# Yuliang-Eliott/Alpha-Multi-factor-models

Measured on AMD Instinct MI355X. Metric: asset-days/sec, factor build+XS regression+KKT (10k assets x 20y), 1/2/4/8 GPU, higher is better.
Workload: dtype f64

## Files before the change

alpha-multi-factor-models_amd/afm/_lib.py:

```python
from __future__ import annotations

import contextlib
import ctypes
import operator
import os
import threading

HERE = os.path.dirname(os.path.abspath(__file__))
LIB_PATH = os.environ.get("AFM_LIB") or os.path.join(HERE, "libafm.so")

P = ctypes.c_void_p
I64 = ctypes.c_int64
I32 = ctypes.c_int
DBL = ctypes.c_double

SIGNATURES = {
    "afm_ctx_create": ("status", "int ptr"),
    "afm_ctx_set_stream": ("status", "ctx ptr"),
    "afm_ctx_set_option": ("status", "ctx str i64"),
    "afm_ctx_get_option": ("status", "ctx str host:i64*"),
    "afm_stream_create_cu_mask": ("status", "int ptr int ptr"),
    "afm_stream_destroy": ("status", "ptr"),
    "afm_ctx_destroy": ("status", "ctx"),
    "afm_last_error": ("str", ""),
# ... 15 lines not shown
    "afm_drop_last_obs_bits_range": ("status", "ctx i64 i64 i64* i64* i64* i64 i64"),
    "afm_factors_part_words": ("i64", "ctx i64 i64 i64 i64"),
    "afm_factors_range_part_f64": ("status", "ctx i64 i64 i64 i64 i64 f64* f64* i64* f64* f64* "
                                             "i64*"),
    "afm_factor_masks_f64": ("status", "ctx i64 i64 i64 i64 i64 i64* i64* i64* i64*"),
    "afm_predict_f64": ("status", "ctx f64* i64 i64 i64 i64 i32* int f64* i64 i64* int f64*"),
    "afm_fama_macbeth_f64": ("status", "ctx f64* i32* i64 int f64* f64*"),
    "afm_ols_residual_f64": ("status", "ctx f64* i64 int int f64* f64* f64*"),
    "afm_vec_add_f64": ("status", "ctx i64 f64* f64*"),
    "afm_ols_intercept_f64": ("status", "ctx int f64* f64*"),
    "afm_lasso_cd_f64": ("status", "ctx f64* int f64 f64 int f64 int f64* f64*"),
    "afm_talib_factors_f64": ("status", "ctx i64 i64 i64 f64* f64* i64* f64*"),
    "afm_ffill_f64": ("status", "ctx i64 i64 i64 f64* i64*"),
    "afm_date_mean_fill_f64": ("status", "ctx i64 i64 i64 i64 f64* i64* f64*"),
    "afm_group_demean_f64": ("status", "ctx i64 i64* i64 f64* f64* f64*"),
    "afm_rebalance_f64": ("status", "ctx i64 i64 i64 i32* i64 f64* i64* f64* i64* i64 i64 i64 f64* "
                                    "f64* int f64 f64 i32* i32* f64* f64* i32* i64* i32*"),
    "afm_pnl_scan_f64": ("status", "ctx i64 i32* i32* f64* i32* i64* f64 f64 f64* f64* f64* f64*"),
    "afm_bootstrap_pnl_f64": ("status", "ctx i64 i32* i64 f64* i32* i32* f64* i64 i64 i32* f64 f64 "
                                        "f64* f64* f64* f64*"),
    "afm_min_variance_weights_f64": ("status", "ctx f64* i64 i64 int f64 f64 f64* f64* i32*"),
    "afm_fwd_returns_f64": ("status", "ctx i64 i64 f64* i64* f64*"),
    "afm_xs_prepare_f64": ("status", "ctx i64 i64 i64 f64* f64* f64* f64* i32* i32*"),
    "afm_xs_prepare_range_f64": ("status", "ctx i64 i64 i64 i64 i64 f64* f64* f64* f64* i32* i32*"),
    "afm_xs_rank_f64": ("status", "ctx i64 i64 f64* i32* i64* i32* i32* i32*"),
    "afm_xs_layers_f64": ("status", "ctx i64 i64 f64* i32* i64* i32* i32* i32*"),
    "afm_xs_stats_f64": ("status", "ctx i64 i64 i32* i64 f64* i32* i32* i32* int f64* f64* i32* "
                                   "f64*"),
    "afm_xs_series_f64": ("status", "ctx i64 f64* f64* f64* i32* int int f64* f64* f64* f64* f64*"),
    "afm_zscore_stats_f64": ("status", "ctx f64* i64 i64 i64 i32* int i64* i64 i64 f64* f64*"),
    "afm_zscore_stats_slab_f64": ("status", "ctx f64* i64 i64 i64 i32* int i64* i64 i64 f64* int "
                                            "int f64* f64*"),
    "afm_zscore_apply_f64": ("status", "ctx f64* i64 i64 i64 i32* int i64* i64 i64 f64* f64* f64* "
                                       "i64 i32* i64*"),
    "afm_zgram_part_bytes": ("int", "int"),
    "afm_zstats_finalize_f64": ("status", "ctx f64* f64* int i64 f64* i32*"),
    "afm_row_bits": ("status", "ctx i64 i64 i64* i64* i32* i64 i64 i64*"),
    "afm_zgram_f64": ("status", "ctx f64* i64 i64 i32* i32* int int f64* int i64* i64 i64 int i64 "
                                "i64 i64 f64* int"),
    "afm_zpool_f64": ("status", "ctx f64* i64 i64 i32* i32* int int f64* int i64* i64 i64 i64 int "
                                "i64 int f64* int"),
    "afm_gram_tree_f64": ("status", "ctx int f64* i64 int int f64*"),
    "afm_zpredict_f64": ("status", "ctx f64* i64 i64 i64 i64 i32* int f64* f64* i64* f64*"),
    "afm_lasso_fit_f64": ("status", "ctx f64* f64* int f64 int f64 int f64* f64*"),
    "afm_lasso_batch_f64": ("status", "ctx f64* i64 f64* i64 int f64* int i64 int int f64 int f64* "
                                      "f64*"),
    "afm_gram_score_f64": ("status", "ctx f64* i64 f64* i64 int f64* int i64 f64*"),
}
SIGNATURES_MV = {
    "afm_rebalance_mv_f64": ("status", "ctx i64 i64 i64 i32* i64 f64* i64* f64* i64* i64 i64 i64 "
                                       "f64* f64* int f64 f64 f64* f64 i32* i32* f64* f64* i32* "
                                       "i64* i32*"),
    "afm_mean_variance_weights_f64": ("status", "ctx f64* i64 i64 int f64* f64 f64 f64 f64* f64* "
                                                "i32*"),
}
SIGNATURES_SCREEN = {
    "afm_screen_ic_f64": ("status", "ctx f64* i64 i64 i64 i32* int f64* i32* i32* i64 f64* i32* "
                                    "i32* f64*"),
    "afm_screen_summary_f64": ("status", "ctx f64* i64 int i32* int int f64* f64* f64*"),
}
TABLES = (SIGNATURES, SIGNATURES_MV, SIGNATURES_SCREEN)
SIGNATURES_RANK = {
    "afm_rank_scratch_words": ("i64", "i64"),
    "afm_rank_returns_f64": ("status", "ctx i64 i64 i32* i64 f64* i32* i32* i64* i64*"),
    "afm_screen_rank_ic_f64": ("status", "ctx f64* i64 i64 i64 i32* int f64* i32* i32* i64 f64* "
                                         "i32* i32* i32* i64* i64* f64*"),
}
ALL_TABLES = TABLES + (SIGNATURES_RANK,)
SIGNATURES_SEAMS = {
    "afm_gram_tree3_f64": ("status", "ctx int f64* int int int int int f64*"),
    "afm_gram_final_f64": ("status", "ctx int f64* int f64* int f64* f64*"),
    "afm_ols_solve_parts_f64": ("status", "ctx f64* int f64* int i64 f64 f64* f64* i32*"),
    "afm_factors_rows_f64": ("status", "ctx i64 i64 i64 f64* f64* f64* f64* i64* f64* i64* i64* "
                                       "i64* i64*"),
    "afm_zstats_rows_f64": ("status", "ctx f64* f64* int i64 f64* i32* i64 i64* i64 i64 i64*"),
}
LOADED_TABLES = ALL_TABLES + (SIGNATURES_SEAMS,)
SIGNATURES_LAYERS = {
    "afm_screen_layers_f64": ("status", "ctx f64* i64 i64 i64 i32* int f64* i32* i32* i64 f64* i32* "
                                        "i32* f64* i32* f64* f64*"),
    "afm_screen_layer_series_f64": ("status", "ctx i64 int f64* f64* f64* f64* f64*"),
}
BOUND_TABLES = LOADED_TABLES + (SIGNATURES_LAYERS,)
_RESTYPE = {"status": I32, "int": I32, "i64": I64, "str": ctypes.c_char_p}
_ARGTYPE = {"int": I32, "i64": I64, "f64": DBL, "str": ctypes.c_char_p}


class AfmError(RuntimeError):
    pass


_lib = None
_lock = threading.Lock()


def lib():
    global _lib
    if _lib is None:
        with _lock:
            if _lib is None:
                if not os.path.exists(LIB_PATH):
                    raise ImportError(f"{LIB_PATH} is not built: run `make -C "
                                      f"{os.path.dirname(HERE)}` (hipcc, gfx950)")
                L = ctypes.CDLL(LIB_PATH)
                for table in BOUND_TABLES:
                    for name, (res, params) in table.items():
                        f = getattr(L, name)
                        f.restype = _RESTYPE[res]
                        f.argtypes = [_ARGTYPE.get(t, P) for t in params.split()]
                _lib = L
    return _lib


def check(rc: int, what: str = ""):
    if rc != 0:
        msg = lib().afm_last_error().decode(errors="replace")
        raise AfmError(f"{what or 'afm'} failed ({rc}): {msg}")


def _as_given(a):
    return a


def _device_buffer(dtype, device: int, where: str):
    import torch

    def conv(t):
        if t is None:
            return None
        if not isinstance(t, torch.Tensor):
            raise AfmError(f"{where}: expected a {dtype} tensor or None, got {type(t).__name__}")
        if t.get_device() != device or t.dtype is not dtype or not t.is_contiguous():
            raise AfmError(f"{where}: expected a contiguous {dtype} tensor on cuda:{device}, got "
                           f"{t.dtype} on {t.device}, contiguous={t.is_contiguous()}")
        return t.data_ptr()
    return conv


def _plans(device: int) -> dict:
    import torch
    scalar = {"int": operator.index, "i64": operator.index, "f64": float}
    buffer = {"f64*": torch.float64, "i32*": torch.int32, "i64*": torch.int64}
    negative = (0).__gt__
    failed = {"status": bool, "int": negative, "i64": negative, "str": lambda s: s is None}
    plans = {}
    for name, (res, params) in (item for table in BOUND_TABLES for item in table.items()):
        toks = params.split()
        takes_ctx = toks[:1] == ["ctx"]
        convs = tuple(_device_buffer(buffer[t], device, f"{name} argument {i}") if t in buffer
                      else scalar.get(t, _as_given)
                      for i, t in enumerate(toks[takes_ctx:], 1))
        plans[name] = (takes_ctx, convs, failed[res])
    return plans


class Context:

    _by_device: dict = {}

    def __init__(self, device: int):
        self.device = device
        h = P()
        check(lib().afm_ctx_create(device, ctypes.byref(h)), "afm_ctx_create")
        self.handle = h
        self._plans = _plans(device)

    def call(self, name: str, *args):
        takes_ctx, convs, failed = self._plans[name]
        if len(args) != len(convs):
            raise TypeError(f"{name} takes {len(convs)} arguments ({len(args)} given)")
        cargs = [cv(a) for cv, a in zip(convs, args)]
        fn = getattr(lib(), name)
        rc = fn(self.handle, *cargs) if takes_ctx else fn(*cargs)
        if failed(rc):
            raise AfmError(f"{name} failed ({rc}): "
                           f"{lib().afm_last_error().decode(errors='replace')}")
        return rc

    @classmethod
    def get(cls, device: int | None = None) -> "Context":
        import torch
        if not torch.cuda.is_available():
            raise AfmError("no GPU visible: the afm engine runs on MI355X only (no CPU fallback)")
        if device is None:
            device = torch.cuda.current_device()
        ctx = cls._by_device.get(device)
        if ctx is None:
            ctx = cls._by_device[device] = Context(device)
        return ctx

    def set_option(self, name: str, value: int):
        self.call("afm_ctx_set_option", name.encode(), int(value))

    def get_option(self, name: str) -> int:
        v = I64()
        self.call("afm_ctx_get_option", name.encode(), ctypes.byref(v))
        return int(v.value)

    def bind_stream(self):
        import torch
        s = torch.cuda.current_stream(self.device).cuda_stream
        check(lib().afm_ctx_set_stream(self.handle, P(s)), "afm_ctx_set_stream")
        return self.handle

    @contextlib.contextmanager
    def on(self, stream):
        import torch
        try:
            with torch.cuda.stream(stream):
                yield self.bind_stream()
        finally:
            self.bind_stream()


def ptr(t) -> P:
    if not t.is_contiguous():
        raise AfmError("tensor must be contiguous")
    return P(t.data_ptr())


def run(name: str, *args, device: int | None = None):
    if device is None:
        device = next((a.device.index for a in args if hasattr(a, "data_ptr")), None)
    ctx = Context.get(device)
    ctx.bind_stream()
    return ctx.call(name, *args)


def factor_names() -> list:
# ... 54 lines not shown
```

alpha-multi-factor-models_amd/csrc/zgram.hip:

```cpp
#include "afm_internal.h"
#include "afm_seams.h"
#include "zgram_layout.h"

#include <cstdlib>

#pragma clang fp contract(off)

namespace afm {
namespace {

typedef double d4 __attribute__((ext_vector_type(4)));
typedef unsigned long long u64;
typedef __attribute__((address_space(3))) double lds_double;

constexpr int kZRS = 66;
constexpr int kZMaxSlots = 3;
constexpr int kZLds = 160 * 1024 - 256;
constexpr int kZProd = 8;
constexpr int kZThreads = 13 * 64;
#ifndef AFM_ZG2_NCW
#define AFM_ZG2_NCW 3
#endif

template <int NT>
struct ZCfg {
    static constexpr int NP = NT * (NT + 1) / 2;
    static constexpr int PE = NP * 256;
    static constexpr int NCW = NT == 7 ? 4 : AFM_ZG2_NCW;
    static constexpr bool BORDER = NT == 7;
    static constexpr int NMP = BORDER ? (NT - 1) * NT / 2 : NP;
    static constexpr int NWAIT = NCW + (BORDER ? 1 : 0);
    static constexpr int KMAX = NT == 7 ? 108 : 16 * NT;
    static constexpr int MC = (KMAX + kZProd - 1) / kZProd;
    static constexpr int q0(int cw) {
        return BORDER ? (cw == 0 ? 0 : 3 + 6 * (cw - 1)) : cw * ((NMP + NCW - 1) / NCW);
    }
    static constexpr int nq(int cw) {
        return BORDER ? (cw == 0 ? 3 : 6)
                      : (q0(cw) + (NMP + NCW - 1) / NCW <= NMP ? (NMP + NCW - 1) / NCW : NMP - q0(cw));
    }
};

template <int NT>
struct ZPairs {
    int I[ZCfg<NT>::NP], J[ZCfg<NT>::NP];
    constexpr ZPairs() : I(), J() {
        int q = 0;
        for (int j = 0; j < NT; ++j)
            for (int i = 0; i <= j; ++i) { I[q] = i; J[q] = j; ++q; }
    }
};

struct ZGramArgs {
    const double* base;
    int64_t col_stride;
    int64_t lda;
    const int32_t* cols;
    const int32_t* zcols;
    int p;
    int ycol;
    int zid;
    const double* zs;
    const uint64_t* bits;
    int64_t t0, nt;
    int mode;
    int nblk;
    int64_t blk0;
    int64_t blk_assets;
    int64_t a_end;
    int nrb;
    int nchunk;
    double* part;
    int even;
};

struct ZSmem {
    lds_double* tile;
    int slot_elems;
    int nslots;
    int ready[kZMaxSlots];
    int freed[kZMaxSlots];
};

__device__ __forceinline__ int lds_load_acq(int* p) {
    return __hip_atomic_load(p, __ATOMIC_ACQUIRE, __HIP_MEMORY_SCOPE_WORKGROUP);
}
__device__ __forceinline__ void wait_count(int* p, int target) {
    while (__builtin_amdgcn_readfirstlane(lds_load_acq(p)) < target) __builtin_amdgcn_s_sleep(1);
}
__device__ __forceinline__ void signal_count(int* p, int lane) {
    asm volatile("s_waitcnt lgkmcnt(0)" ::: "memory");
    if (lane == 0) __hip_atomic_fetch_add(p, 1, __ATOMIC_RELEASE, __HIP_MEMORY_SCOPE_WORKGROUP);
}

struct Seq {
    int item, nitems, stride;
    int t, a_lo;
    int masked;
    int k, kend, kreal;
    __device__ void start(const ZGramArgs& g) {
        if (g.mode == 0) {
            const int d = item / g.nblk, b = item - d * g.nblk;
            t = (int)g.t0 + d;
            const int lo = (int)g.blk0 + b * (int)g.blk_assets;
            int hi = lo + (int)g.blk_assets;
            if (hi > (int)g.a_end) hi = (int)g.a_end;
            const int n = hi > lo ? (hi - lo + 63) / 64 : 0;
            a_lo = lo;
            k = 0;
            kreal = n;
            kend = (n > 0 ? n : 1) + (g.even ? ((n > 0 ? n : 1) & 1) : 0);
        } else {
            const int r = item / g.nchunk, c = item - r * g.nchunk;
            const int c0 = (int)g.t0 + (int)(((int64_t)c * g.nt) / g.nchunk);
            const int c1 = (int)g.t0 + (int)(((int64_t)(c + 1) * g.nt) / g.nchunk);
            const int n = c1 > c0 ? c1 - c0 : 1;
            a_lo = (int)g.blk0 + r * 64;
            k = c0;
            kreal = c1;
            kend = c0 + n + (g.even ? (n & 1) : 0);
            t = c0;
        }
        masked = k >= kreal ? 1 : 0;
    }
    __device__ void init(const ZGramArgs& g) {
        stride = gridDim.x;
        nitems = g.mode == 0 ? (int)g.nt * g.nblk : g.nrb * g.nchunk;
        item = blockIdx.x;
        if (item < nitems) start(g);
    }
    __device__ bool valid() const { return item < nitems; }
    __device__ bool last() const { return k + 1 == kend; }
    __device__ int row_asset(int lane) const { return a_lo + lane; }
    __device__ void advance(const ZGramArgs& g) {
        if (k + 1 < kend) {
            ++k;
            masked = k >= kreal ? 1 : 0;
            if (g.mode == 0) a_lo += 64;
            else t = masked ? t : k;
            return;
        }
        item += stride;
        if (item < nitems) start(g);
    }
};

template <int NT, int MODE, bool ZS>
__device__ void zgram_produce(const ZGramArgs& g, ZSmem& sm, const int lane, const int pw) {
    constexpr int MC = ZCfg<NT>::MC;
    const int p = g.p;
    const int K = p + 2;
    const int lda = (int)g.lda;
    int pk[MC];
#pragma unroll
    for (int j = 0; j < MC; ++j) {
        const int k = pw + kZProd * j;
        const bool feat = k >= 1 && k <= p;
        const int pl = feat ? g.cols[k - 1] : g.ycol;
        const int zr = feat ? (g.zcols ? g.zcols[k - 1] : k - 1) : g.zid;
        pk[j] = __builtin_amdgcn_readfirstlane(pl | (zr << 16));
    }
    auto xsrc = [&](int j) {
        int q = pk[j];
        asm volatile("" : "+s"(q));
        return reinterpret_cast<const char*>(g.base + (int64_t)(q & 0xffff) * g.col_stride);
    };
    auto zsrc = [&](int j) {
        int q = pk[j];
        asm volatile("" : "+s"(q));
        return (unsigned)((q >> 16) * lda) * 16u;
    };
    const char* zb = reinterpret_cast<const char*>(g.zs);
    struct Buf {
        double x[MC];
        bool ok;
        unsigned zoff;
        int item;
    };
    Buf A, C;
    double mu[MC], rs[MC];
    int zitem = -1;
    Seq cur;
    cur.init(g);
    auto xload = [&](Buf& B) {
        const int t = cur.t;
        const int a = cur.row_asset(lane);
        const bool in = a < (int)g.a_end && !cur.masked;
        const int ac = in ? a : 0;
        B.ok = in && ((g.bits[(int64_t)(t >> 6) * lda + ac] >> (t & 63)) & 1ull);
        B.zoff = (unsigned)ac * 16u;
        B.item = cur.item;
        const unsigned off = (unsigned)(t * lda + ac) * 8u;
#pragma unroll
        for (int j = 0; j < MC; ++j) B.x[j] = *reinterpret_cast<const double*>(xsrc(j) + off);
    };
    auto zload = [&](const unsigned zoff) {
        if (!ZS) return;
#pragma unroll
        for (int j = 0; j < MC; ++j) {
            const double2 m = *reinterpret_cast<const double2*>(zb + zsrc(j) + zoff);
            mu[j] = m.x;
            rs[j] = m.y;
        }
    };
    int slot = 0, gen = 0;
    auto stage = [&](const Buf& B) {
        if (ZS && MODE == 1 && B.item != zitem) {
            zload(B.zoff);
            zitem = B.item;
        }
        wait_count(&sm.freed[slot], ZCfg<NT>::NWAIT * gen);
        lds_double* tb = sm.tile + slot * sm.slot_elems + lane;
#pragma unroll
        for (int j = 0; j < MC; ++j) {
            const int k = pw + kZProd * j;
            const int lrow = k < K ? k : p + 3;
            double v = ZS ? (B.x[j] - mu[j]) * rs[j] : B.x[j];
            if (k == 0) v = 1.0;
            tb[lrow * kZRS] = B.ok ? v : 0.0;
        }
        signal_count(&sm.ready[slot], lane);
        if (++slot == sm.nslots) { slot = 0; ++gen; }
    };
    bool ha = cur.valid(), hc = false;
    if (ha) { xload(A); cur.advance(g); }
    if (MODE == 0 && ha) zload(A.zoff);
    hc = cur.valid();
    if (hc) { xload(C); cur.advance(g); }
    while (ha) {
        stage(A);
        if (MODE == 0 && hc) zload(C.zoff);
        ha = cur.valid();
        if (ha) { xload(A); cur.advance(g); }
        if (!hc) break;
        stage(C);
        if (MODE == 0 && ha) zload(A.zoff);
        hc = cur.valid();
        if (hc) { xload(C); cur.advance(g); }
    }
}

template <int NT, int MODE, bool ZS>
__device__ void zgram_produce_pairs(const ZGramArgs& g, ZSmem& sm, const int lane, const int pw) {
    constexpr int MC = ZCfg<NT>::MC;
    const int p = g.p;
    const int K = p + 2;
    const int lda = (int)g.lda;
    int pk[MC];
#pragma unroll
    for (int j = 0; j < MC; ++j) {
        const int k = pw + kZProd * j;
        const bool feat = k >= 1 && k <= p;
        const int pl = feat ? g.cols[k - 1] : g.ycol;
        const int zr = feat ? (g.zcols ? g.zcols[k - 1] : k - 1) : g.zid;
        pk[j] = __builtin_amdgcn_readfirstlane(pl | (zr << 16));
    }
    auto xsrc = [&](int j) {
        int q = pk[j];
        asm volatile("" : "+s"(q));
        return reinterpret_cast<const char*>(g.base + (int64_t)(q & 0xffff) * g.col_stride);
    };
    auto zsrc = [&](int j) {
        int q = pk[j];
        asm volatile("" : "+s"(q));
        return (unsigned)((q >> 16) * lda) * 16u;
    };
    const char* zb = reinterpret_cast<const char*>(g.zs);
    struct Buf {
        double x[MC];
        uint32_t word;
        bool in, valid;
        unsigned zoff;
        int t, item;
    };
    Buf A, C;
    double mu[MC], rs[MC];
    Seq cur;
    cur.init(g);
    auto xload = [&](Buf& B) {
        const bool v = cur.valid();
        const int a = cur.row_asset(lane);
        const bool in = v && !cur.masked && a < (int)g.a_end;
        const int ac = in ? a : 0, tl = in ? cur.t : 0;
        B.valid = v;
        B.in = in;
        B.t = cur.t;
        B.item = v ? cur.item : -1;
        B.zoff = (unsigned)ac * 16u;
        B.word = reinterpret_cast<const uint32_t*>(g.bits)[((int64_t)(tl >> 6) * lda + ac) * 2 +
                                                           ((tl >> 5) & 1)];
        const unsigned off = (unsigned)(tl * lda + ac) * 8u;
#pragma unroll
        for (int j = 0; j < MC; ++j) B.x[j] = *reinterpret_cast<const double*>(xsrc(j) + off);
        if (v) cur.advance(g);
    };
    auto zload = [&](const unsigned zoff) {
        if (!ZS) return;
#pragma unroll
        for (int j = 0; j < MC; ++j) {
            const double2 m = *reinterpret_cast<const double2*>(zb + zsrc(j) + zoff);
            mu[j] = m.x;
            rs[j] = m.y;
        }
    };
    int slot = 0, gen = 0;
    auto stage = [&](const Buf& B) {
        wait_count(&sm.freed[slot], ZCfg<NT>::NWAIT * gen);
        lds_double* tb = sm.tile + slot * sm.slot_elems + lane;
        const bool ok = B.in && ((B.word >> (B.t & 31)) & 1u);
#pragma unroll
        for (int j = 0; j < MC; ++j) {
            const int k = pw + kZProd * j;
            const int lrow = k < K ? k : p + 3;
            double v = ZS ? (B.x[j] - mu[j]) * rs[j] : B.x[j];
            if (k == 0) v = 1.0;
            tb[lrow * kZRS] = ok ? v : 0.0;
        }
        signal_count(&sm.ready[slot], lane);
        if (++slot == sm.nslots) { slot = 0; ++gen; }
    };
    xload(A);
    if (MODE == 0) zload(A.zoff);
    xload(C);
    while (A.valid) {
        if (MODE == 1) zload(A.zoff);
        const int item = A.item;
        do {
            stage(A);
            if (MODE == 0) zload(C.zoff);
            xload(A);
            stage(C);
            if (MODE == 0) zload(A.zoff);
            xload(C);
        } while (A.valid && A.item == item);
    }
}

template <int NT, int CW>
__device__ void zgram_consume(const ZGramArgs& g, ZSmem& sm, const int lane) {
    using Cf = ZCfg<NT>;
    constexpr ZPairs<NT> tab{};
    constexpr int Q0 = Cf::q0(CW);
    constexpr int NQ = Cf::nq(CW);
    constexpr int THI = tab.J[Q0 + NQ - 1] + 1;
    const int fi = lane & 15, kk = lane >> 4;
    const int p = g.p;
    int lrow[NT];
#pragma unroll
    for (int t = 0; t < NT; ++t) {
        const int f = t * 16 + fi;
        lrow[t] = f <= p + 1 ? f : p + 2;
    }
    d4 acc[NQ];
#pragma unroll
    for (int q = 0; q < NQ; ++q) acc[q] = d4{0.0, 0.0, 0.0, 0.0};
    int slot = 0, gen = 1;
    Seq cur;
    for (cur.init(g); cur.valid(); cur.advance(g)) {
        wait_count(&sm.ready[slot], kZProd * gen);
        const lds_double* tb = sm.tile + slot * sm.slot_elems;
        double fa[NT], fb[NT];
        auto ld = [&](double (&f)[NT], int it) {
            const int a = it * 4 + kk;
#pragma unroll
            for (int t = 0; t < THI; ++t) f[t] = tb[lrow[t] * kZRS + a];
        };
        auto step = [&](const double (&f)[NT]) {
#pragma unroll
            for (int q = 0; q < NQ; ++q)
                acc[q] = __builtin_amdgcn_mfma_f64_16x16x4f64(f[tab.I[Q0 + q]], f[tab.J[Q0 + q]],
                                                              acc[q], 0, 0, 0);
        };
        ld(fa, 0);
#pragma unroll
        for (int it = 0; it < 16; it += 2) {
            ld(fb, it + 1);
            step(fa);
            if (it + 2 < 16) ld(fa, it + 2);
            step(fb);
        }
        signal_count(&sm.freed[slot], lane);
        if (++slot == sm.nslots) { slot = 0; ++gen; }
        if (cur.last()) {
            double* out = g.part + (int64_t)cur.item * Cf::PE + Q0 * 256 + lane;
#pragma unroll
            for (int q = 0; q < NQ; ++q) {
#pragma unroll
                for (int r = 0; r < 4; ++r) out[(q * 4 + r) * 64] = acc[q][r];
                acc[q] = d4{0.0, 0.0, 0.0, 0.0};
            }
        }
    }
}

__device__ __forceinline__ double rdlane_d(double v, int l) {
    const long long b = __double_as_longlong(v);
    const int lo = __builtin_amdgcn_readlane((int)b, l);
    const int hi = __builtin_amdgcn_readlane((int)(b >> 32), l);
    return __longlong_as_double(((long long)hi << 32) | (unsigned)lo);
}

template <int NT, int NB>
__device__ void zgram_border(const ZGramArgs& g, ZSmem& sm, const int lane) {
    constexpr ZPairs<NT> tab{};
    const int K = g.p + 2;
    double acc[2][NB];
#pragma unroll
    for (int cc = 0; cc < 2; ++cc)
#pragma unroll
        for (int b = 0; b < NB; ++b) acc[cc][b] = 0.0;
    int slot = 0, gen = 1;
    Seq cur;
    for (cur.init(g); cur.valid(); cur.advance(g)) {
        wait_count(&sm.ready[slot], kZProd * gen);
        const lds_double* tb = sm.tile + slot * sm.slot_elems;
        const lds_double* c0 = tb + lane * kZRS;
        const lds_double* c1 = tb + (lane + 64 < K ? lane + 64 : g.p + 2) * kZRS;
        const lds_double* bb = tb + 96 * kZRS;
#pragma unroll 8
        for (int r = 0; r < 64; ++r) {
            const double x0 = c0[r], x1 = c1[r];
#pragma unroll
            for (int b = 0; b < NB; ++b) {
                const double zb = bb[b * kZRS + r];
                acc[0][b] = __builtin_fma(x0, zb, acc[0][b]);
                acc[1][b] = __builtin_fma(x1, zb, acc[1][b]);
            }
        }
        signal_count(&sm.freed[slot], lane);
        if (++slot == sm.nslots) { slot = 0; ++gen; }
        if (cur.last()) {
            double* out = g.part + (int64_t)cur.item * ZCfg<NT>::PE;
#pragma unroll
            for (int cc = 0; cc < 2; ++cc) {
                const int c = lane + 64 * cc;
                if (c < K) {
                    const int ti = c >> 4, w = c & 15;
                    int q = 0;
#pragma unroll
                    for (int qq = 0; qq < ZCfg<NT>::NP; ++qq)
                        if (tab.I[qq] == ti && tab.J[qq] == NT - 1) q = qq;
                    const int r4 = w >> 2, lrow = (w & 3) * 16;
#pragma unroll
                    for (int b = 0; b < NB; ++b) out[q * 256 + r4 * 64 + lrow + b] = acc[cc][b];
                }
#pragma unroll
                for (int b = 0; b < NB; ++b) acc[cc][b] = 0.0;
            }
        }
    }
}

template <int NT>
__device__ void zgram_border_any(const ZGramArgs& g, ZSmem& sm, const int lane) {
    switch (g.p + 2 - 96) {
        case 1: zgram_border<NT, 1>(g, sm, lane); break;
        case 2: zgram_border<NT, 2>(g, sm, lane); break;
        case 3: zgram_border<NT, 3>(g, sm, lane); break;
        case 4: zgram_border<NT, 4>(g, sm, lane); break;
        case 5: zgram_border<NT, 5>(g, sm, lane); break;
        case 6: zgram_border<NT, 6>(g, sm, lane); break;
        case 7: zgram_border<NT, 7>(g, sm, lane); break;
        case 8: zgram_border<NT, 8>(g, sm, lane); break;
        case 9: zgram_border<NT, 9>(g, sm, lane); break;
        case 10: zgram_border<NT, 10>(g, sm, lane); break;
        case 11: zgram_border<NT, 11>(g, sm, lane); break;
        case 12: zgram_border<NT, 12>(g, sm, lane); break;
        default: zgram_border<NT, 0>(g, sm, lane); break;
    }
}

template <int NT, int MODE, bool ZS>
__global__ __launch_bounds__(kZThreads, 1) void zgram_kernel(ZGramArgs g, int nslots) {
    extern __shared__ __attribute__((aligned(16))) double ring[];
    __shared__ ZSmem sm;
    const int tid = threadIdx.x, lane = tid & 63;
    const int wave = __builtin_amdgcn_readfirstlane(tid >> 6);
    const int se = (g.p + 4) * kZRS;
    for (int i = tid; i < nslots * se; i += kZThreads) ring[i] = 0.0;
    if (tid == 0) {
        sm.tile = (lds_double*)ring;
        sm.slot_elems = se;
        sm.nslots = nslots;
    }
    if (tid < kZMaxSlots) { sm.ready[tid] = 0; sm.freed[tid] = 0; }
    __syncthreads();
    if (wave >= 4 && wave < 4 + kZProd) {
        __builtin_amdgcn_s_setprio(1);
        if (NT == 2) zgram_produce_pairs<NT, MODE, ZS>(g, sm, lane, wave - 4);
        else zgram_produce<NT, MODE, ZS>(g, sm, lane, wave - 4);
        return;
    }
    if (wave == 12) {
        __builtin_amdgcn_s_setprio(2);
        if constexpr (ZCfg<NT>::BORDER) zgram_border_any<NT>(g, sm, lane);
        return;
// ... 182 lines not shown
__global__ __launch_bounds__(256) void zpredict_kernel(const double* base, int64_t col_stride,
                                                       int64_t lda, int64_t t0, int64_t nt,
                                                       const int32_t* cols, int p,
                                                       const double* zs, const double* beta,
                                                       const uint64_t* bits, double* pred) {
    __shared__ int sj[kPredMaxP];
    __shared__ double sb[kPredMaxP];
    __shared__ int snnz;
    const int tid = threadIdx.x;
    if (tid < 64) {
        int cnt = 0;
        for (int j0 = 0; j0 < p; j0 += 64) {
            const int j = j0 + tid;
            const double bj = j < p ? beta[1 + j] : 0.0;
            const u64 m = __ballot(bj != 0.0);
            if (bj != 0.0) {
                const int pos = cnt + __popcll(m & ((1ull << tid) - 1ull));
                sj[pos] = j;
                sb[pos] = bj;
            }
            cnt += __popcll(m);
        }
        if (tid == 0) snnz = cnt;
    }
    __syncthreads();
    const int nnz = snnz;
    const int64_t a = (int64_t)blockIdx.x * 64 + (tid & 63);
    const int64_t t = t0 + (int64_t)blockIdx.y * 4 + (tid >> 6);
    if (t >= t0 + nt) return;
    const bool use = (bits[(t >> 6) * lda + a] >> (t & 63)) & 1ull;
    double v = __builtin_nan("");
    if (use) {
        double s = beta[0];
        const double* cell = base + t * lda + a;
        for (int q = 0; q < nnz; ++q) {
            const int j = sj[q];
            const double2 m = reinterpret_cast<const double2*>(zs)[(int64_t)j * lda + a];
            const double z = (cell[(int64_t)cols[j] * col_stride] - m.x) * m.y;
            s = s + sb[q] * z;
        }
        v = s;
    }
    pred[t * lda + a] = v;
}

}
}

using namespace afm;

extern "C" int afm_zgram_part_bytes(int p) {
    return (int)sizeof(double) * (zgram_nt(p) == 2 ? ZCfg<2>::PE : ZCfg<7>::PE);
}

template <int NT, int MODE, bool ZS>
static int launch_zgram(afm_ctx* ctx, const ZGramArgs& g, int64_t nitems, int grid) {
    int64_t wg = grid > 0 ? grid : 256;
    if (wg > nitems) wg = nitems;
    if (wg <= 0) return AFM_OK;
    const int slot_bytes = (int)sizeof(double) * (g.p + 4) * kZRS;
    int nslots = kZLds / slot_bytes;
    if (nslots > kZMaxSlots) nslots = kZMaxSlots;
    AFM_CHECK_ARG(nslots >= 2, "ring does not fit in LDS");
    AFM_HIP(afm_lds_opt_in(ctx, (const void*)zgram_kernel<NT, MODE, ZS>, kZLds));
    hipLaunchKernelGGL((zgram_kernel<NT, MODE, ZS>), dim3((unsigned)wg), dim3(kZThreads),
                       (size_t)nslots * slot_bytes, ctx->stream, g, nslots);
    AFM_HIP(hipGetLastError());
    return AFM_OK;
}

static int zgram_common_checks(const double* base, const int32_t* cols, const double* zs,
                               const uint64_t* bits, double* part, int p, int64_t lda,
                               int64_t a_end, int64_t blk0, int64_t t0, int64_t nt) {
    AFM_CHECK_ARG(base && cols && bits && part, "null buffer");
    AFM_CHECK_ARG(p >= 1 && p + 2 <= ZCfg<7>::KMAX, "need 1 <= p <= 106");
    AFM_CHECK_ARG(lda > 0 && lda % 64 == 0 && a_end <= lda, "lda must be a multiple of 64 >= a_end");
    AFM_CHECK_ARG(blk0 >= 0 && blk0 % 64 == 0, "blk0 must be a multiple of 64");
    AFM_CHECK_ARG(t0 >= 0 && nt >= 0, "bad date range");
    AFM_CHECK_ARG((t0 + nt) * lda * 8 < (int64_t)1 << 32 && lda * 16 * 112 < (int64_t)1 << 32,
                  "plane too large for 32-bit offsets");
    return AFM_OK;
}

extern "C" int afm_zgram_f64(afm_ctx* ctx, const double* base, int64_t col_stride, int64_t lda,
                             const int32_t* cols, const int32_t* zcols, int p, int ycol,
                             const double* zs, int zid, const uint64_t* bits, int64_t t0,
                             int64_t nt, int nblk, int64_t blk0, int64_t blk_assets,
                             int64_t a_end, double* part, int grid) {
    AFM_CTX(ctx);
    const int rc = zgram_common_checks(base, cols, zs, bits, part, p, lda, a_end, blk0, t0, nt);
    if (rc) return rc;
    AFM_CHECK_ARG(nblk >= 1 && blk_assets > 0 && blk_assets % 64 == 0 && nt * nblk < (1ll << 31),
                  "blocks must be 64-aligned");
    if (nt == 0) return AFM_OK;
    const int even = (!zs || zgram_nt(p) == 2) ? 1 : 0;
    ZGramArgs g{base, col_stride, lda, cols, zcols, p, ycol, zid, zs, bits, t0, nt, 0, nblk, blk0,
                blk_assets, a_end, 0, 1, part, even};
    if (!zs) return launch_zgram<2, 0, false>(ctx, g, nt * nblk, grid);
    return zgram_nt(p) == 2 ? launch_zgram<2, 0, true>(ctx, g, nt * nblk, grid)
                            : launch_zgram<7, 0, true>(ctx, g, nt * nblk, grid);
}

extern "C" int afm_zpool_f64(afm_ctx* ctx, const double* base, int64_t col_stride, int64_t lda,
                             const int32_t* cols, const int32_t* zcols, int p, int ycol,
                             const double* zs, int zid, const uint64_t* bits, int64_t t0,
                             int64_t nt, int64_t blk0, int nrb, int64_t a_end, int nchunk,
                             double* part, int grid) {
    AFM_CTX(ctx);
    const int rc = zgram_common_checks(base, cols, zs, bits, part, p, lda, a_end, blk0, t0, nt);
    if (rc) return rc;
    AFM_CHECK_ARG(nrb >= 0 && nchunk >= 1 && (int64_t)nrb * nchunk < (1ll << 31), "bad leaves");
    if (nrb == 0) return AFM_OK;
    ZGramArgs g{base, col_stride, lda, cols, zcols, p, ycol, zid, zs, bits, t0, nt, 1, 1, blk0,
                64, a_end, nrb, nchunk, part, zgram_nt(p) == 2 ? 1 : 0};
    AFM_CHECK_ARG(zs != nullptr, "afm_zpool_f64 needs zs");
    return zgram_nt(p) == 2 ? launch_zgram<2, 1, true>(ctx, g, (int64_t)nrb * nchunk, grid)
                            : launch_zgram<7, 1, true>(ctx, g, (int64_t)nrb * nchunk, grid);
}

extern "C" int afm_gram_tree_f64(afm_ctx* ctx, int p, const double* in, int64_t total, int per,
                                 int final_out, double* out) {
    AFM_CTX(ctx);
    AFM_CHECK_ARG(in && out, "null buffer");
    AFM_CHECK_ARG(per >= 1 && per <= 32 && total >= 0, "need 1 <= per <= 32");
    AFM_CHECK_ARG(p >= 1 && p + 2 <= ZCfg<7>::KMAX, "need 1 <= p <= 106");
    if (total == 0) return AFM_OK;
    const unsigned ng = (unsigned)((total + per - 1) / per);
    if (zgram_nt(p) == 2)
        hipLaunchKernelGGL(tree_merge_kernel<2>, dim3(ng, 1), dim3(256), 0, ctx->stream, in, total,
                           per, final_out, p + 2, out);
    else
        hipLaunchKernelGGL(tree_merge_kernel<7>, dim3(ng, 4), dim3(256), 0, ctx->stream, in, total,
                           per, final_out, p + 2, out);
    AFM_HIP(hipGetLastError());
    return AFM_OK;
}

extern "C" int afm_gram_tree3_f64(afm_ctx* ctx, int p, const double* leaves, int nrb, int c1,
                                  int c2, int rb_per_blk, int nblk, double* out) {
    AFM_CTX(ctx);
    AFM_CHECK_ARG(leaves && out, "null buffer");
    AFM_CHECK_ARG(p >= 1 && p + 2 <= ZCfg<7>::KMAX, "need 1 <= p <= 106");
    AFM_CHECK_ARG(nrb >= 0 && nblk >= 0, "bad leaf counts");
    AFM_CHECK_ARG(c1 >= 1 && c1 <= 32 && c2 >= 1 && c2 <= 32 && rb_per_blk >= 1 &&
                      rb_per_blk <= 32 && c2 * rb_per_blk <= kT3Items,
                  "need 1 <= c1, c2, rb_per_blk <= 32 and c2 * rb_per_blk <= 64");
    AFM_CHECK_ARG((int64_t)nblk * rb_per_blk >= nrb, "nblk blocks do not hold nrb row-blocks");
    if (nblk == 0) return AFM_OK;
    if (zgram_nt(p) == 2)
        hipLaunchKernelGGL(tree3_kernel<2>, dim3(ZCfg<2>::PE / 64, (unsigned)nblk),
                           dim3(kT3Waves * 64), 0, ctx->stream, leaves, nrb, c1, c2, rb_per_blk,
                           out);
    else
        hipLaunchKernelGGL(tree3_kernel<7>, dim3(ZCfg<7>::PE / 64, (unsigned)nblk),
                           dim3(kT3Waves * 64), 0, ctx->stream, leaves, nrb, c1, c2, rb_per_blk,
                           out);
    AFM_HIP(hipGetLastError());
    return AFM_OK;
}

extern "C" int afm_gram_final_f64(afm_ctx* ctx, int p, const double* blocks, int nblk,
                                  const double* te_leaves, int nte, double* gram,
                                  double* te_gram) {
    AFM_CTX(ctx);
    AFM_CHECK_ARG(blocks && gram, "null buffer");
    AFM_CHECK_ARG(p >= 1 && p + 2 <= ZCfg<7>::KMAX, "need 1 <= p <= 106");
    AFM_CHECK_ARG(nblk >= 1 && nblk <= 32, "need 1 <= nblk <= 32");
    AFM_CHECK_ARG(!te_leaves || (te_gram && nte >= 1 && nte <= 32),
                  "te_leaves need te_gram and 1 <= nte <= 32");
    if (zgram_nt(p) == 2)
        hipLaunchKernelGGL(gram_final_kernel<2>, dim3(ZCfg<2>::PE / 256), dim3(256), 0,
                           ctx->stream, blocks, nblk, te_leaves, nte, p + 2, gram, te_gram);
    else
        hipLaunchKernelGGL(gram_final_kernel<7>, dim3(ZCfg<7>::PE / 256), dim3(256), 0,
                           ctx->stream, blocks, nblk, te_leaves, nte, p + 2, gram, te_gram);
    AFM_HIP(hipGetLastError());
    return AFM_OK;
}

extern "C" int afm_zstats_rows_f64(afm_ctx* ctx, const double* mu, const double* sd, int K,
                                   int64_t lda, double* zs, int32_t* asset_ok, int64_t nch,
                                   const uint64_t* rows, int64_t t0, int64_t t1, uint64_t* out) {
    AFM_CTX(ctx);
// ... 47 lines not shown
```

alpha-multi-factor-models_amd/csrc/zgram_layout.h:

```cpp
#pragma once
#include <hip/hip_runtime.h>

#pragma clang fp contract(off)

namespace afm {

constexpr int zgram_nt(int p) { return p + 2 <= 32 ? 2 : 7; }
constexpr int zgram_pe(int nt) { return nt * (nt + 1) / 2 * 256; }

__device__ __forceinline__ void zgram_elem_rc(int e, int& row, int& col) {
    int i = e >> 8, j = 0;
    while (i > j) { i -= j + 1; ++j; }
    const int r = (e >> 6) & 3, lane = e & 63;
    row = i * 16 + (lane >> 4) + 4 * r;
    col = j * 16 + (lane & 15);
}

__device__ __forceinline__ double zgram_tree32(double (&v)[32], int n) {
#pragma unroll
    for (int s = 1; s < 32; s *= 2)
#pragma unroll
        for (int i = 0; i + s < 32; i += 2 * s)
            if (i + s < n) v[i] = v[i] + v[i + s];
    return v[0];
}

}
```

Before: 1.563 billion.

## Stage multiple 64-row blocks per LDS ring slot in the small-p Gram kernel

```diff
diff --git a/alpha-multi-factor-models_amd/afm/_lib.py b/alpha-multi-factor-models_amd/afm/_lib.py
--- a/alpha-multi-factor-models_amd/afm/_lib.py
+++ b/alpha-multi-factor-models_amd/afm/_lib.py
@@ -121,6 +121,12 @@
     "afm_screen_layer_series_f64": ("status", "ctx i64 int f64* f64* f64* f64* f64*"),
 }
 BOUND_TABLES = LOADED_TABLES + (SIGNATURES_LAYERS,)
+SIGNATURES_ZSLOTS = {
+    "afm_zgram_slots_f64": ("status", "ctx f64* i64 i64 i32* i32* int int f64* int i64* i64 i64 int "
+                                      "i64 i64 i64 f64* int int"),
+    "afm_zgram_slot_plan": ("i64", "i64 int i64 i64 i64 int int int host:i32* i64"),
+}
+CALL_TABLES = BOUND_TABLES + (SIGNATURES_ZSLOTS,)
 _RESTYPE = {"status": I32, "int": I32, "i64": I64, "str": ctypes.c_char_p}
 _ARGTYPE = {"int": I32, "i64": I64, "f64": DBL, "str": ctypes.c_char_p}
 
@@ -142,7 +148,7 @@
                     raise ImportError(f"{LIB_PATH} is not built: run `make -C "
                                       f"{os.path.dirname(HERE)}` (hipcc, gfx950)")
                 L = ctypes.CDLL(LIB_PATH)
-                for table in BOUND_TABLES:
+                for table in CALL_TABLES:
                     for name, (res, params) in table.items():
                         f = getattr(L, name)
                         f.restype = _RESTYPE[res]
@@ -183,7 +189,7 @@
     negative = (0).__gt__
     failed = {"status": bool, "int": negative, "i64": negative, "str": lambda s: s is None}
     plans = {}
-    for name, (res, params) in (item for table in BOUND_TABLES for item in table.items()):
+    for name, (res, params) in (item for table in CALL_TABLES for item in table.items()):
         toks = params.split()
         takes_ctx = toks[:1] == ["ctx"]
         convs = tuple(_device_buffer(buffer[t], device, f"{name} argument {i}") if t in buffer
diff --git a/alpha-multi-factor-models_amd/csrc/zgram.hip b/alpha-multi-factor-models_amd/csrc/zgram.hip
--- a/alpha-multi-factor-models_amd/csrc/zgram.hip
+++ b/alpha-multi-factor-models_amd/csrc/zgram.hip
@@ -1,5 +1,6 @@
 #include "afm_internal.h"
 #include "afm_seams.h"
+#include "afm_zgram_slots.h"
 #include "zgram_layout.h"
 
 #include <cstdlib>
@@ -51,28 +52,7 @@
     }
 };
 
-struct ZGramArgs {
-    const double* base;
-    int64_t col_stride;
-    int64_t lda;
-    const int32_t* cols;
-    const int32_t* zcols;
-    int p;
-    int ycol;
-    int zid;
-    const double* zs;
-    const uint64_t* bits;
-    int64_t t0, nt;
-    int mode;
-    int nblk;
-    int64_t blk0;
-    int64_t blk_assets;
-    int64_t a_end;
-    int nrb;
-    int nchunk;
-    double* part;
-    int even;
-};
+using Seq = ZSeq<1>;
 
 struct ZSmem {
     lds_double* tile;
@@ -93,58 +73,6 @@
     if (lane == 0) __hip_atomic_fetch_add(p, 1, __ATOMIC_RELEASE, __HIP_MEMORY_SCOPE_WORKGROUP);
 }
 
-struct Seq {
-    int item, nitems, stride;
-    int t, a_lo;
-    int masked;
-    int k, kend, kreal;
-    __device__ void start(const ZGramArgs& g) {
-        if (g.mode == 0) {
-            const int d = item / g.nblk, b = item - d * g.nblk;
-            t = (int)g.t0 + d;
-            const int lo = (int)g.blk0 + b * (int)g.blk_assets;
-            int hi = lo + (int)g.blk_assets;
-            if (hi > (int)g.a_end) hi = (int)g.a_end;
-            const int n = hi > lo ? (hi - lo + 63) / 64 : 0;
-            a_lo = lo;
-            k = 0;
-            kreal = n;
-            kend = (n > 0 ? n : 1) + (g.even ? ((n > 0 ? n : 1) & 1) : 0);
-        } else {
-            const int r = item / g.nchunk, c = item - r * g.nchunk;
-            const int c0 = (int)g.t0 + (int)(((int64_t)c * g.nt) / g.nchunk);
-            const int c1 = (int)g.t0 + (int)(((int64_t)(c + 1) * g.nt) / g.nchunk);
-            const int n = c1 > c0 ? c1 - c0 : 1;
-            a_lo = (int)g.blk0 + r * 64;
-            k = c0;
-            kreal = c1;
-            kend = c0 + n + (g.even ? (n & 1) : 0);
-            t = c0;
-        }
-        masked = k >= kreal ? 1 : 0;
-    }
-    __device__ void init(const ZGramArgs& g) {
-        stride = gridDim.x;
-        nitems = g.mode == 0 ? (int)g.nt * g.nblk : g.nrb * g.nchunk;
-        item = blockIdx.x;
-        if (item < nitems) start(g);
-    }
-    __device__ bool valid() const { return item < nitems; }
-    __device__ bool last() const { return k + 1 == kend; }
-    __device__ int row_asset(int lane) const { return a_lo + lane; }
-    __device__ void advance(const ZGramArgs& g) {
-        if (k + 1 < kend) {
-            ++k;
-            masked = k >= kreal ? 1 : 0;
-            if (g.mode == 0) a_lo += 64;
-            else t = masked ? t : k;
-            return;
-        }
-        item += stride;
-        if (item < nitems) start(g);
-    }
-};
-
 template <int NT, int MODE, bool ZS>
 __device__ void zgram_produce(const ZGramArgs& g, ZSmem& sm, const int lane, const int pw) {
     constexpr int MC = ZCfg<NT>::MC;
@@ -181,7 +109,7 @@
     double mu[MC], rs[MC];
     int zitem = -1;
     Seq cur;
-    cur.init(g);
+    cur.init(g, blockIdx.x, gridDim.x);
     auto xload = [&](Buf& B) {
         const int t = cur.t;
         const int a = cur.row_asset(lane);
@@ -276,7 +204,7 @@
     Buf A, C;
     double mu[MC], rs[MC];
     Seq cur;
-    cur.init(g);
+    cur.init(g, blockIdx.x, gridDim.x);
     auto xload = [&](Buf& B) {
         const bool v = cur.valid();
         const int a = cur.row_asset(lane);
@@ -356,7 +284,7 @@
     for (int q = 0; q < NQ; ++q) acc[q] = d4{0.0, 0.0, 0.0, 0.0};
     int slot = 0, gen = 1;
     Seq cur;
-    for (cur.init(g); cur.valid(); cur.advance(g)) {
+    for (cur.init(g, blockIdx.x, gridDim.x); cur.valid(); cur.advance(g)) {
         wait_count(&sm.ready[slot], kZProd * gen);
         const lds_double* tb = sm.tile + slot * sm.slot_elems;
         double fa[NT], fb[NT];
@@ -393,6 +321,198 @@
     }
 }
 
+template <int R>
+constexpr int zslot_rs() { return 64 * R + 2; }
+
+template <int R, bool ZS>
+__device__ void zgram_produce_wide(const ZGramArgs& g, ZSmem& sm, const int lane, const int pw) {
+    static_assert(R >= 2 && R % 2 == 0, "a slot is staged as buffer pairs");
+    constexpr int MC = ZCfg<2>::MC;
+    constexpr int RS = zslot_rs<R>();
+    const int p = g.p;
+    const int K = p + 2;
+    const int lda = (int)g.lda;
+    int pk[MC];
+#pragma unroll
+    for (int j = 0; j < MC; ++j) {
+        const int k = pw + kZProd * j;
+        const bool feat = k >= 1 && k <= p;
+        const int pl = feat ? g.cols[k - 1] : g.ycol;
+        const int zr = feat ? (g.zcols ? g.zcols[k - 1] : k - 1) : g.zid;
+        pk[j] = __builtin_amdgcn_readfirstlane(pl | (zr << 16));
+    }
+    auto xsrc = [&](int j) {
+        int q = pk[j];
+        asm volatile("" : "+s"(q));
+        return reinterpret_cast<const char*>(g.base + (int64_t)(q & 0xffff) * g.col_stride);
+    };
+    auto zsrc = [&](int j) {
+        int q = pk[j];
+        asm volatile("" : "+s"(q));
+        return (unsigned)((q >> 16) * lda) * 16u;
+    };
+    const char* zb = reinterpret_cast<const char*>(g.zs);
+    struct Buf {
+        double x[MC];
+        uint32_t word;
+        bool in, valid;
+        unsigned zoff;
+        int t;
+    };
+    Buf A, C;
+    double mu[MC], rs[MC];
+    ZSeq<R> cur;
+    cur.init(g, blockIdx.x, gridDim.x);
+    auto xload = [&](Buf& B, const int j) {
+        const bool v = cur.valid();
+        const int a = cur.row_asset(lane) + 64 * j;
+        const bool in = v && !cur.masked && a < cur.a_hi;
+        const int ac = in ? a : 0, tl = in ? cur.t : 0;
+        B.valid = v;
+        B.in = in;
+        B.t = cur.t;
+        B.zoff = (unsigned)ac * 16u;
+        B.word = reinterpret_cast<const uint32_t*>(g.bits)[((int64_t)(tl >> 6) * lda + ac) * 2 +
+                                                           ((tl >> 5) & 1)];
+        const unsigned off = (unsigned)(tl * lda + ac) * 8u;
+#pragma unroll
+        for (int c = 0; c < MC; ++c) B.x[c] = *reinterpret_cast<const double*>(xsrc(c) + off);
+        if (j == R - 1 && v) cur.advance(g);
+    };
+    auto zload = [&](const unsigned zoff) {
+        if (!ZS) return;
+#pragma unroll
+        for (int c = 0; c < MC; ++c) {
+            const double2 m = *reinterpret_cast<const double2*>(zb + zsrc(c) + zoff);
+            mu[c] = m.x;
+            rs[c] = m.y;
+        }
+    };
+    int slot = 0, gen = 0;
+    auto stage = [&](const Buf& B, const int j) {
+        if (j == 0) wait_count(&sm.freed[slot], ZCfg<2>::NWAIT * gen);
+        lds_double* tb = sm.tile + slot * sm.slot_elems + j * 64 + lane;
+        const bool ok = B.in && ((B.word >> (B.t & 31)) & 1u);
+#pragma unroll
+        for (int c = 0; c < MC; ++c) {
+            const int k = pw + kZProd * c;
+            const int lrow = k < K ? k : p + 3;
+            double v = ZS ? (B.x[c] - mu[c]) * rs[c] : B.x[c];
+            if (k == 0) v = 1.0;
+            tb[lrow * RS] = ok ? v : 0.0;
+        }
+        if (j == R - 1) {
+            signal_count(&sm.ready[slot], lane);
+            if (++slot == sm.nslots) { slot = 0; ++gen; }
+        }
+    };
+    xload(A, 0);
+    zload(A.zoff);
+    xload(C, 1);
+    while (A.valid) {
+#pragma unroll
+        for (int j = 0; j < R; j += 2) {
+            stage(A, j);
+            zload(C.zoff);
+            xload(A, (j + 2) % R);
+            stage(C, j + 1);
+            zload(A.zoff);
+            xload(C, (j + 3) % R);
+        }
+    }
+}
+
+template <int CW, int R>
+__device__ void zgram_consume_wide(const ZGramArgs& g, ZSmem& sm, const int lane) {
+    constexpr int NT = 2;
+    using Cf = ZCfg<NT>;
+    constexpr ZPairs<NT> tab{};
+    constexpr int RS = zslot_rs<R>();
+    constexpr int Q0 = Cf::q0(CW);
+    constexpr int NQ = Cf::nq(CW);
+    constexpr int THI = tab.J[Q0 + NQ - 1] + 1;
+    const int fi = lane & 15, kk = lane >> 4;
+    const int p = g.p;
+    int lrow[NT];
+#pragma unroll
+    for (int t = 0; t < NT; ++t) {
+        const int f = t * 16 + fi;
+        lrow[t] = f <= p + 1 ? f : p + 2;
+    }
+    d4 acc[NQ];
+#pragma unroll
+    for (int q = 0; q < NQ; ++q) acc[q] = d4{0.0, 0.0, 0.0, 0.0};
+    int slot = 0, gen = 1;
+    ZSeq<R> cur;
+    for (cur.init(g, blockIdx.x, gridDim.x); cur.valid(); cur.advance(g)) {
+        wait_count(&sm.ready[slot], kZProd * gen);
+        const lds_double* tb = sm.tile + slot * sm.slot_elems;
+        const int nr = __builtin_amdgcn_readfirstlane(cur.masked ? 0 : cur.real_blocks());
+        double fa[NT], fb[NT];
+        auto ld = [&](double (&f)[NT], int a0, int it) {
+            const int a = a0 + it * 4 + kk;
+#pragma unroll
+            for (int t = 0; t < THI; ++t) f[t] = tb[lrow[t] * RS + a];
+        };
+        auto step = [&](const double (&f)[NT]) {
+#pragma unroll
+            for (int q = 0; q < NQ; ++q)
+                acc[q] = __builtin_amdgcn_mfma_f64_16x16x4f64(f[tab.I[Q0 + q]], f[tab.J[Q0 + q]],
+                                                              acc[q], 0, 0, 0);
+        };
+#pragma unroll
+        for (int j = 0; j < R; ++j) {
+            if (j < nr) {
+                ld(fa, j * 64, 0);
+#pragma unroll
+                for (int it = 0; it < 16; it += 2) {
+                    ld(fb, j * 64, it + 1);
+                    step(fa);
+                    if (it + 2 < 16) ld(fa, j * 64, it + 2);
+                    step(fb);
+                }
+            }
+        }
+        signal_count(&sm.freed[slot], lane);
+        if (++slot == sm.nslots) { slot = 0; ++gen; }
+        if (cur.last()) {
+            double* out = g.part + (int64_t)cur.item * Cf::PE + Q0 * 256 + lane;
+#pragma unroll
+            for (int q = 0; q < NQ; ++q) {
+#pragma unroll
+                for (int r = 0; r < 4; ++r) out[(q * 4 + r) * 64] = acc[q][r];
+                acc[q] = d4{0.0, 0.0, 0.0, 0.0};
+            }
+        }
+    }
+}
+
+template <bool ZS, int R>
+__global__ __launch_bounds__(kZThreads, 1) void zgram_slots_kernel(ZGramArgs g, int nslots) {
+    extern __shared__ __attribute__((aligned(16))) double ring[];
+    __shared__ ZSmem sm;
+    static_assert(ZCfg<2>::NCW == 3 && !ZCfg<2>::BORDER, "three consumer waves, no border wave");
+    const int tid = threadIdx.x, lane = tid & 63;
+    const int wave = __builtin_amdgcn_readfirstlane(tid >> 6);
+    const int se = (g.p + 4) * zslot_rs<R>();
+    for (int i = tid; i < nslots * se; i += kZThreads) ring[i] = 0.0;
+    if (tid == 0) {
+        sm.tile = (lds_double*)ring;
+        sm.slot_elems = se;
+        sm.nslots = nslots;
+    }
+    if (tid < kZMaxSlots) { sm.ready[tid] = 0; sm.freed[tid] = 0; }
+    __syncthreads();
+    if (wave >= 4 && wave < 4 + kZProd) {
+        __builtin_amdgcn_s_setprio(1);
+        zgram_produce_wide<R, ZS>(g, sm, lane, wave - 4);
+        return;
+    }
+    if (wave == 0) zgram_consume_wide<0, R>(g, sm, lane);
+    else if (wave == 1) zgram_consume_wide<1, R>(g, sm, lane);
+    else if (wave == 2) zgram_consume_wide<2, R>(g, sm, lane);
+}
+
 __device__ __forceinline__ double rdlane_d(double v, int l) {
     const long long b = __double_as_longlong(v);
     const int lo = __builtin_amdgcn_readlane((int)b, l);
@@ -411,7 +531,7 @@
         for (int b = 0; b < NB; ++b) acc[cc][b] = 0.0;
     int slot = 0, gen = 1;
     Seq cur;
-    for (cur.init(g); cur.valid(); cur.advance(g)) {
+    for (cur.init(g, blockIdx.x, gridDim.x); cur.valid(); cur.advance(g)) {
         wait_count(&sm.ready[slot], kZProd * gen);
         const lds_double* tb = sm.tile + slot * sm.slot_elems;
         const lds_double* c0 = tb + lane * kZRS;
@@ -760,23 +880,107 @@
     return AFM_OK;
 }
 
+#ifndef AFM_ZG2_WSLOTS
+#define AFM_ZG2_WSLOTS 2
+#endif
+constexpr int kZWideSlots = AFM_ZG2_WSLOTS;
+static_assert(kZWideSlots >= 2 && kZWideSlots <= kZMaxSlots, "ring depth");
+template <bool ZS, int R>
+static int launch_zgram_slots(afm_ctx* ctx, const ZGramArgs& g, int64_t nitems, int grid) {
+    int64_t wg = grid > 0 ? grid : 256;
+    if (wg > nitems) wg = nitems;
+    if (wg <= 0) return AFM_OK;
+    const int slot_bytes = (int)sizeof(double) * (g.p + 4) * zslot_rs<R>();
+    int nslots = kZLds / slot_bytes;
+    if (nslots > kZWideSlots) nslots = kZWideSlots;
+    AFM_CHECK_ARG(nslots >= 2, "ring does not fit in LDS");
+    AFM_HIP(afm_lds_opt_in(ctx, (const void*)zgram_slots_kernel<ZS, R>, kZLds));
+    hipLaunchKernelGGL((zgram_slots_kernel<ZS, R>), dim3((unsigned)wg), dim3(kZThreads),
+                       (size_t)nslots * slot_bytes, ctx->stream, g, nslots);
+    AFM_HIP(hipGetLastError());
+    return AFM_OK;
+}
+
+#ifndef AFM_ZG2_RPS
+#define AFM_ZG2_RPS 2
+#endif
+static int zgram_rps(int nt, int rps) {
+    if (rps == 0) return nt == 2 ? AFM_ZG2_RPS : 1;
+    if (rps == 1 || (nt == 2 && (rps == 2 || rps == 4))) return rps;
+    return 0;
+}
+
+extern "C" int afm_zgram_slots_f64(afm_ctx* ctx, const double* base, int64_t col_stride,
+                                   int64_t lda, const int32_t* cols, const int32_t* zcols, int p,
+                                   int ycol, const double* zs, int zid, const uint64_t* bits,
+                                   int64_t t0, int64_t nt, int nblk, int64_t blk0,
+                                   int64_t blk_assets, int64_t a_end, double* part, int grid,
+                                   int rps) {
+    AFM_CTX(ctx);
+    const int rc = zgram_common_checks(base, cols, zs, bits, part, p, lda, a_end, blk0, t0, nt);
+    if (rc) return rc;
+    AFM_CHECK_ARG(nblk >= 1 && blk_assets > 0 && blk_assets % 64 == 0 && nt * nblk < (1ll << 31),
+                  "blocks must be 64-aligned");
+    const int ntile = zs ? zgram_nt(p) : 2;
+    AFM_CHECK_ARG(zs || p + 2 <= ZCfg<2>::KMAX, "raw columns need p <= 30");
+    const int R = zgram_rps(ntile, rps);
+    AFM_CHECK_ARG(R != 0, "rps must be 0, 1, or (p <= 30) 2 or 4");
+    if (nt == 0) return AFM_OK;
+    const int even = ntile == 2 && R == 1 ? 1 : 0;
+    ZGramArgs g{base, col_stride, lda, cols, zcols, p, ycol, zid, zs, bits, t0, nt, 0, nblk, blk0,
+                blk_assets, a_end, 0, 1, part, even};
+    const int64_t nitems = nt * nblk;
+    if (!zs) {
+        if (R == 4) return launch_zgram_slots<false, 4>(ctx, g, nitems, grid);
+        if (R == 2) return launch_zgram_slots<false, 2>(ctx, g, nitems, grid);
+        return launch_zgram<2, 0, false>(ctx, g, nitems, grid);
+    }
+    if (ntile == 7) return launch_zgram<7, 0, true>(ctx, g, nitems, grid);
+    if (R == 4) return launch_zgram_slots<true, 4>(ctx, g, nitems, grid);
+    if (R == 2) return launch_zgram_slots<true, 2>(ctx, g, nitems, grid);
+    return launch_zgram<2, 0, true>(ctx, g, nitems, grid);
+}
+
 extern "C" int afm_zgram_f64(afm_ctx* ctx, const double* base, int64_t col_stride, int64_t lda,
                              const int32_t* cols, const int32_t* zcols, int p, int ycol,
                              const double* zs, int zid, const uint64_t* bits, int64_t t0,
                              int64_t nt, int nblk, int64_t blk0, int64_t blk_assets,
                              int64_t a_end, double* part, int grid) {
-    AFM_CTX(ctx);
-    const int rc = zgram_common_checks(base, cols, zs, bits, part, p, lda, a_end, blk0, t0, nt);
-    if (rc) return rc;
-    AFM_CHECK_ARG(nblk >= 1 && blk_assets > 0 && blk_assets % 64 == 0 && nt * nblk < (1ll << 31),
-                  "blocks must be 64-aligned");
-    if (nt == 0) return AFM_OK;
-    const int even = (!zs || zgram_nt(p) == 2) ? 1 : 0;
-    ZGramArgs g{base, col_stride, lda, cols, zcols, p, ycol, zid, zs, bits, t0, nt, 0, nblk, blk0,
-                blk_assets, a_end, 0, 1, part, even};
-    if (!zs) return launch_zgram<2, 0, false>(ctx, g, nt * nblk, grid);
-    return zgram_nt(p) == 2 ? launch_zgram<2, 0, true>(ctx, g, nt * nblk, grid)
-                            : launch_zgram<7, 0, true>(ctx, g, nt * nblk, grid);
+    return afm_zgram_slots_f64(ctx, base, col_stride, lda, cols, zcols, p, ycol, zs, zid, bits, t0,
+                               nt, nblk, blk0, blk_assets, a_end, part, grid, 0);
+}
+
+template <int R>
+static int64_t slot_plan(const ZGramArgs& g, int grid, int wg, int32_t* out, int64_t cap) {
+    int64_t n = 0;
+    ZSeq<R> cur;
+    for (cur.init(g, wg, grid); cur.valid(); cur.advance(g)) {
+        const int nr = cur.masked ? 0 : cur.real_blocks();
+        for (int j = 0; j < R; ++j, ++n)
+            if (out && n < cap) {
+                out[3 * n] = cur.t;
+                out[3 * n + 1] = cur.a_lo + 64 * j;
+                out[3 * n + 2] = j < nr ? 1 : 0;
+            }
+    }
+    return n;
+}
+
+extern "C" int64_t afm_zgram_slot_plan(int64_t nt, int nblk, int64_t blk0, int64_t blk_assets,
+                                       int64_t a_end, int rps, int grid, int wg, int32_t* out,
+                                       int64_t cap) {
+    const int R = zgram_rps(2, rps);
+    if (nt < 0 || nblk < 1 || blk0 < 0 || blk0 % 64 || blk_assets <= 0 || blk_assets % 64 ||
+        nt * nblk >= (1ll << 31) || R == 0 || grid < 0 || wg < 0 || cap < 0)
+        return -1;
+    int64_t ngrid = grid > 0 ? grid : 256;
+    if (ngrid > nt * nblk) ngrid = nt * nblk;
+    if (wg >= ngrid) return 0;
+    ZGramArgs g{nullptr, 0, 0, nullptr, nullptr, 0, 0, 0, nullptr, nullptr, 0, nt, 0, nblk, blk0,
+                blk_assets, a_end, 0, 1, nullptr, R == 1 ? 1 : 0};
+    return R == 4 ? slot_plan<4>(g, (int)ngrid, wg, out, cap)
+         : R == 2 ? slot_plan<2>(g, (int)ngrid, wg, out, cap)
+                  : slot_plan<1>(g, (int)ngrid, wg, out, cap);
 }
 
 extern "C" int afm_zpool_f64(afm_ctx* ctx, const double* base, int64_t col_stride, int64_t lda,
diff --git a/alpha-multi-factor-models_amd/csrc/zgram_layout.h b/alpha-multi-factor-models_amd/csrc/zgram_layout.h
--- a/alpha-multi-factor-models_amd/csrc/zgram_layout.h
+++ b/alpha-multi-factor-models_amd/csrc/zgram_layout.h
@@ -1,5 +1,7 @@
 #pragma once
 #include <hip/hip_runtime.h>
+
+#include <cstdint>
 
 #pragma clang fp contract(off)
 
@@ -25,4 +27,87 @@
     return v[0];
 }
 
+struct ZGramArgs {
+    const double* base;
+    int64_t col_stride;
+    int64_t lda;
+    const int32_t* cols;
+    const int32_t* zcols;
+    int p;
+    int ycol;
+    int zid;
+    const double* zs;
+    const uint64_t* bits;
+    int64_t t0, nt;
+    int mode;
+    int nblk;
+    int64_t blk0;
+    int64_t blk_assets;
+    int64_t a_end;
+    int nrb;
+    int nchunk;
+    double* part;
+    int even;
+};
+
+template <int RPS>
+struct ZSeq {
+    int item, nitems, stride;
+    int t, a_lo;
+    int a_hi;
+    int masked;
+    int k, kend, kreal;
+    __host__ __device__ void start(const ZGramArgs& g) {
+        if (g.mode == 0) {
+            const int d = item / g.nblk, b = item - d * g.nblk;
+            t = (int)g.t0 + d;
+            const int lo = (int)g.blk0 + b * (int)g.blk_assets;
+            int hi = lo + (int)g.blk_assets;
+            if (hi > (int)g.a_end) hi = (int)g.a_end;
+            const int n = hi > lo ? ((hi - lo + 63) / 64 + RPS - 1) / RPS : 0;
+            a_lo = lo;
+            a_hi = hi;
+            k = 0;
+            kreal = n;
+            kend = (n > 0 ? n : 1) + (g.even ? ((n > 0 ? n : 1) & 1) : 0);
+        } else {
+            const int r = item / g.nchunk, c = item - r * g.nchunk;
+            const int c0 = (int)g.t0 + (int)(((int64_t)c * g.nt) / g.nchunk);
+            const int c1 = (int)g.t0 + (int)(((int64_t)(c + 1) * g.nt) / g.nchunk);
+            const int n = c1 > c0 ? c1 - c0 : 1;
+            a_lo = (int)g.blk0 + r * 64;
+            a_hi = (int)g.a_end;
+            k = c0;
+            kreal = c1;
+            kend = c0 + n + (g.even ? (n & 1) : 0);
+            t = c0;
+        }
+        masked = k >= kreal ? 1 : 0;
+    }
+    __host__ __device__ void init(const ZGramArgs& g, int first, int step) {
+        stride = step;
+        nitems = g.mode == 0 ? (int)g.nt * g.nblk : g.nrb * g.nchunk;
+        item = first;
+        if (item < nitems) start(g);
+    }
+    __host__ __device__ bool valid() const { return item < nitems; }
+    __host__ __device__ bool last() const { return k + 1 == kend; }
+    __host__ __device__ int row_asset(int lane) const { return a_lo + lane; }
+    __host__ __device__ int real_blocks() const {
+        const int n = a_hi > a_lo ? (a_hi - a_lo + 63) / 64 : 0;
+        return n < RPS ? n : RPS;
+    }
+    __host__ __device__ void advance(const ZGramArgs& g) {
+        if (k + 1 < kend) {
+            ++k;
+            masked = k >= kreal ? 1 : 0;
+            if (g.mode == 0) a_lo += 64 * RPS;
+            else t = masked ? t : k;
+            return;
+        }
+        item += stride;
+        if (item < nitems) start(g);
+    }
+};
+
 }
diff --git a/include/afm_zgram_slots.h b/include/afm_zgram_slots.h
--- /dev/null
+++ b/include/afm_zgram_slots.h
@@ -0,0 +1,22 @@
+#ifndef AFM_ZGRAM_SLOTS_H
+#define AFM_ZGRAM_SLOTS_H
+
+#include "afm.h"
+
+#ifdef __cplusplus
+extern "C" {
+#endif
+
+int afm_zgram_slots_f64(afm_ctx* ctx, const double* base, int64_t col_stride, int64_t lda,
+                        const int32_t* cols, const int32_t* zcols, int p, int ycol,
+                        const double* zs, int zid, const uint64_t* bits, int64_t t0, int64_t nt,
+                        int nblk, int64_t blk0, int64_t blk_assets, int64_t a_end, double* part,
+                        int grid, int rps);
+int64_t afm_zgram_slot_plan(int64_t nt, int nblk, int64_t blk0, int64_t blk_assets, int64_t a_end,
+                            int rps, int grid, int wg, int32_t* out, int64_t cap);
+
+#ifdef __cplusplus
+}
+#endif
+
+#endif
```

Measured after the change: 1.573 billion (median of 6 runs). About the same (+0.6%).
